# utiasSTARS/pyslam

Hardware: AMD Instinct MI355X
Metric: ms/LM-iter (Jac build + J^T J + Schur solve), stereo BA @ 500k residuals (lower is better)
Workload: dtype f64

## Files before the change

### pyslam_amd/csrc/ps_abi_problem.h

```cpp


const char* ps_last_error(void) { return g_err.c_str(); }

int ps_device_count(void) {
    int n = 0;
    if (hipGetDeviceCount(&n) != hipSuccess) return 0;
    return n;
}

int ps_warm_up(void) {
    static std::once_flag once;
    static int rc = 0;
    std::call_once(once, [] {
        void* p = nullptr;
        if (hipMalloc(&p, 256) != hipSuccess) { rc = fail("hipMalloc failed (no usable HIP device?)"); return; }
        hipLaunchKernelGGL(k_zero4, dim3(1), dim3(256), 0, 0, (size_t)8, (double*)p, (size_t)0, (double*)nullptr, (size_t)0,
                           (double*)nullptr, (size_t)0, (double*)nullptr);
        double hostw[4] = {0, 0, 0, 0};
        (void)hipMemsetAsync(p, 0, 256, 0);
        (void)hipMemcpyAsync((char*)p + 128, p, 64, hipMemcpyDeviceToDevice, 0);
        (void)hipMemcpyAsync(hostw, p, sizeof(hostw), hipMemcpyDeviceToHost, 0);
        if (hipDeviceSynchronize() != hipSuccess) rc = fail("the warm-up launch failed");
        hipFree(p);
        hipFuncAttributes a;
#define PS_TOUCH(...) (void)hipFuncGetAttributes(&a, reinterpret_cast<const void*>(&__VA_ARGS__))
        PS_TOUCH(k_landmark_pass<false>); PS_TOUCH(k_landmark_pass_packed<false, false>); PS_TOUCH(k_landmark_pass_packed<false, true>); PS_TOUCH(k_backsub_packed<false>); PS_TOUCH(k_pose_pass<false>); PS_TOUCH(k_pose_finalize); PS_TOUCH(k_schur_pairs_db<0>);
        PS_TOUCH(k_schur_combine); PS_TOUCH(k_backsub<false>); PS_TOUCH(k_cost_reproj<false>); PS_TOUCH(k_cost_packed<false>); PS_TOUCH(k_reduce3); PS_TOUCH(k_reduce_partials);
        PS_TOUCH(k_copy2); PS_TOUCH(k_zero4); PS_TOUCH(k_lag_status_check);
        PS_TOUCH(k_block_jacobi_factor<6>); PS_TOUCH(k_scale_blocks<6>); PS_TOUCH(k_scale_blocks_p<6>); PS_TOUCH(k_rows_setup<6>);
        PS_TOUCH(k_coarse_rowsums<6>); PS_TOUCH(k_coarse_matrix<6>); PS_TOUCH(k_coarse_chol<6, true>); PS_TOUCH(k_coarse_border<6>);
        PS_TOUCH(k_coarse_mreduce<6>); PS_TOUCH(k_coarse_xbuild<6>); PS_TOUCH(k_coarse_recover<6>); PS_TOUCH(k_cg_fused_lds<6, 8>);
        PS_TOUCH(k_cg_fused<6, 8>); PS_TOUCH(k_cg_unscale<6>); PS_TOUCH(k_update_poses<6>); PS_TOUCH(k_update_points);
        PS_TOUCH(k_xcoarse_rowsums<6>); PS_TOUCH(k_xcoarse_matrix<6>); PS_TOUCH(k_band_chol<6>); PS_TOUCH(k_band_inverse); PS_TOUCH(k_band_inverse_rl<false>);
        PS_TOUCH(k_band_inverse_rl<true>); PS_TOUCH(k_bp_v); PS_TOUCH(k_bp_t); PS_TOUCH(k_bp_w); PS_TOUCH(k_bp_dense_sep); PS_TOUCH(k_bp_dense);
        PS_TOUCH(k_xcg_restrict<6>); PS_TOUCH(k_xcg_f2_coarse<6, 3>); PS_TOUCH(k_xcg_fused1<6, 8, false>); PS_TOUCH(k_xcg_fused1<6, 0, true>);
        PS_TOUCH(k_xcg_fused1<6, 2, false>); PS_TOUCH(k_xcg_fused1<6, 6, false>);
        PS_TOUCH(k_factor_pass<6>); PS_TOUCH(k_factor_assemble<6>); PS_TOUCH(k_cost_factors<6>);
        PS_TOUCH(k_factor_pass<3>); PS_TOUCH(k_factor_assemble<3>); PS_TOUCH(k_cost_factors<3>); PS_TOUCH(k_block_jacobi_factor<3>);
        PS_TOUCH(k_update_poses<3>); PS_TOUCH(k_direct_solve<6>); PS_TOUCH(k_direct_solve<3>);
        PS_TOUCH(k_motion_only_solve<false>); PS_TOUCH(k_motion_only_iteration<false>);
        PS_TOUCH(k_pcg_spmv<6>); PS_TOUCH(k_pcg_spmv<3>); PS_TOUCH(k_ldi_init); PS_TOUCH(k_ldi_update); PS_TOUCH(k_ldi_gemm); PS_TOUCH(k_ldi_mirror);
        PS_TOUCH(k_ldi_ritz); PS_TOUCH(k_ldi_seed_prep); PS_TOUCH(k_ldi_fro_total); PS_TOUCH(k_ldi_pad_identity);
        PS_TOUCH(k_ldi_scaled_dense<6>); PS_TOUCH(k_ldi_sym_unscale<6>); PS_TOUCH(k_ldi_scaled_dense<3>); PS_TOUCH(k_ldi_sym_unscale<3>);
        PS_TOUCH(k_shard_pack<6>); PS_TOUCH(k_shard_unpack<6>); PS_TOUCH(k_publish); PS_TOUCH(k_cov_rhs); PS_TOUCH(k_triangulate<false>);
        PS_TOUCH(k_scale_blocks<3>); PS_TOUCH(k_rows_setup<3>); PS_TOUCH(k_coarse_rowsums<3>); PS_TOUCH(k_coarse_matrix<3>);
        PS_TOUCH(k_coarse_chol<3, true>); PS_TOUCH(k_coarse_border<3>); PS_TOUCH(k_coarse_mreduce<3>); PS_TOUCH(k_coarse_xbuild<3>);
        PS_TOUCH(k_coarse_recover<3>); PS_TOUCH(k_cg_fused_lds<3, 8>); PS_TOUCH(k_cg_unscale<3>);
#undef PS_TOUCH
    });
    return rc;
}

int ps_problem_destroy(ps_problem* h) {
    if (!h) return 0;
    if (h->cp_dbg) {
        long long c[8]; hipMemcpy(c, h->cp_dbg, 64, hipMemcpyDeviceToHost);
        int khz = 100000; hipDeviceGetAttribute(&khz, hipDeviceAttributeWallClockRate, 0);
        fprintf(stderr, "k_cg_persist, workgroup 0, %ld launches, us per launch: recurrences %.2f | sync %.2f | products + publish %.2f | gather %.2f "
                "(%.1f failed passes) | sync %.2f | dots + sync %.2f\n", h->cp_launches, c[0] * 1e3 / khz / h->cp_launches, c[1] * 1e3 / khz / h->cp_launches,
                c[2] * 1e3 / khz / h->cp_launches, c[3] * 1e3 / khz / h->cp_launches, (double)c[7] / h->cp_launches, c[4] * 1e3 / khz / h->cp_launches,
                c[5] * 1e3 / khz / h->cp_launches);
        hipFree(h->cp_dbg);
    }
    if (h->xp_dbg) {
        std::vector<long long> c(3 * 64 * 8); hipMemcpy(c.data(), h->xp_dbg, c.size() * 8, hipMemcpyDeviceToHost);
        int khz = 100000; hipDeviceGetAttribute(&khz, hipDeviceAttributeWallClockRate, 0);
        for (int w = 0; w < 3; ++w) {
            double ph[6] = {0, 0, 0, 0, 0, 0}; int np = 0;
            for (int p = 1; p < 64; ++p) {
                const long long* t = &c[((size_t)w * 64 + p) * 8];
                if (!t[6] || !t[4]) break;
                ph[0] += t[0] - t[6]; ph[1] += t[1] - t[0]; ph[2] += t[2] - t[1]; ph[3] += t[5] - t[2]; ph[4] += t[3] - t[5]; ph[5] += t[4] - t[3]; ++np;
            }
            const double u = 1e3 / khz / std::max(np, 1);
            fprintf(stderr, "k_xcg_persist, workgroup %s, last launch, %d passes, us per pass: t + coarse y %.2f | columns %.2f | products + publish %.2f | "
                    "first gather pass %.2f | rest of the gather %.2f | record sums + dots %.2f | sum %.2f\n", w == 0 ? "0" : (w == 1 ? "nwg/2" : "nwg-1"), np,
                    ph[0] * u, ph[1] * u, ph[2] * u, ph[3] * u, ph[4] * u, ph[5] * u, (ph[0] + ph[1] + ph[2] + ph[3] + ph[4] + ph[5]) * u);
        }
        hipFree(h->xp_dbg);
    }
    if (h->chk_sums) {
        hipDeviceSynchronize();
        fprintf(stderr, "PS_XCG_INV_SUM %p:", (void*)h);
        for (int k = 0; k < std::min(h->chk_nsum, 64); ++k) fprintf(stderr, " [%d use %016llx | side A_c %016llx -> inv %016llx]", k, h->chk_sums[3 * k], h->chk_sums[3 * k + 1], h->chk_sums[3 * k + 2]);
        fprintf(stderr, "\n");
        hipHostFree(h->chk_sums);
    }
    if (h->chk_cnt) {
        int32_t c[4] = {}; hipDeviceSynchronize(); hipMemcpy(c, h->chk_cnt, 16, hipMemcpyDeviceToHost);
        fprintf(stderr, "PS_XCG_AC_CHECK: %d comparisons, entries that differ between the side stream's assembly and the solver stream's: A_c %d, BSZ %d; A_c behind the assembly vs at the end of the side job: %d\n", c[2], c[0], c[1], c[3]);
        hipFree(h->chk_Ac_side); hipFree(h->chk_Ac); hipFree(h->chk_BSZ); hipFree(h->chk_cnt);
    }
    if (ps_env("PS_HOST_TIMING") && h->host_calls)
        fprintf(stderr, "ps_gn_iteration: %ld calls, %.1f us per call on the host, of which %.1f us waiting for the GPU (%ld waits)\n",
                h->host_calls, h->host_call_ns * 1e-3 / h->host_calls, h->host_wait_ns * 1e-3 / h->host_calls, h->host_waits);
    hipStreamSynchronize(h->stream);
    h->persist_release();
    if (h->side) hipStreamSynchronize(h->side);
    if (h->ldi_stream) hipStreamSynchronize(h->ldi_stream);
    cov_release(h);
    if (h->cov_xbuf) hipFree(h->cov_xbuf);
    if (h->tri_buf) hipFree(h->tri_buf);
    for (void* p : h->allocs) hipFree(p);
    h->arena_release();
    for (hipEvent_t e : h->ev_pool) hipEventDestroy(e);
    if (h->ev_ldi) { hipEventDestroy(h->ev_ldi); hipEventDestroy(h->ev_ldi_sread); }
    if (h->ldi_stream && !ps_pool().give(ps_pool().side_streams, h->ldi_stream)) hipStreamDestroy(h->ldi_stream);
    if (h->side) { hipStreamSynchronize(h->side); if (!h->side_poolable || !ps_pool().give(ps_pool().side_streams, h->side)) hipStreamDestroy(h->side); hipEventDestroy(h->ev_ac); hipEventDestroy(h->ev_chol); hipEventDestroy(h->ev_acdone); }
    if (h->own_stream && h->stream && !ps_pool().give(ps_pool().streams, h->stream)) hipStreamDestroy(h->stream);
    delete h;
    return 0;
}

struct DescStage {
    ps_problem_desc d;
    std::vector<std::vector<char>> bufs;
    int pull_bytes(const void** field, size_t bytes) {
        if (!bytes || !*field) return 0;
        bufs.emplace_back(bytes);
        if (hipMemcpy(bufs.back().data(), *field, bytes, hipMemcpyDeviceToHost) != hipSuccess)
            return fail("ps_problem_create: copy of a device-resident table failed (PS_DESC_DEVICE_TABLES set on a host pointer?)");
        *field = bufs.back().data();
        return 0;
    }
    int pull(const double** f, size_t n) { return pull_bytes((const void**)f, n * sizeof(double)); }
    int pull(const int32_t** f, size_t n) { return pull_bytes((const void**)f, n * sizeof(int32_t)); }
    bool obs_pending = false;
    int pull_obs() {
        if (!obs_pending) return 0;
        obs_pending = false;
        const size_t N = (size_t)std::max<int64_t>(0, d.num_obs);
        return pull(&d.obs_pose, N) || pull(&d.obs_point, N) || pull(&d.obs_uvd, 3 * N) || pull(&d.obs_grp, N);
    }
    int stage(const ps_problem_desc* in) {
        d = *in;
        if (!(d.flags & PS_DESC_DEVICE_TABLES)) return 0;
        const size_t P = std::max(0, d.num_poses), L = std::max(0, d.num_points), N = (size_t)std::max<int64_t>(0, d.num_obs);
        const size_t E = (size_t)std::max<int64_t>(0, d.num_edges), Q = (size_t)std::max<int64_t>(0, d.num_priors);
        const size_t X = (size_t)std::max<int64_t>(0, d.num_extra_pairs), PW = d.dof == 6 ? 12 : 6, DD = (size_t)d.dof * d.dof;
        obs_pending = N > 0;
        return pull(&d.pose_rid, P) || pull(&d.point_vid, L) || pull(&d.cams, 5 * (size_t)std::max(0, d.num_cams)) || pull(&d.stiff3, 9 * (size_t)std::max(0, d.num_stiff3)) ||
               pull(&d.obs_groups, 4 * (size_t)std::max(0, d.num_obs_groups)) || pull(&d.e_i, E) || pull(&d.e_j, E) ||
// ... 739 lines not shown
```

### pyslam_amd/csrc/ps_host_cg.h

```cpp

namespace {

struct StageTimer {
    ps_problem* h;
    int stage;
    hipEvent_t a = nullptr, b = nullptr;
    int slot = -1;
    StageTimer(ps_problem* h_, int st, int level = 2) : h(h_), stage(st) {
        if (h->profiling < level) return;
        if (h->profiling == 1 && h->prof_every > 1 &&
            h->prof_tick % h->prof_every != (st == PS_ST_CG_KERNEL ? h->prof_every / 2 : 0)) return;
        if (h->ev_used + 2 > h->ev_pool.size()) {
            for (int i = 0; i < 64; ++i) { hipEvent_t e; hipEventCreate(&e); h->ev_pool.push_back(e); }
        }
        slot = (int)h->ev_used;
        a = h->ev_pool[h->ev_used++];
        b = h->ev_pool[h->ev_used++];
        hipEventRecord(a, h->stream);
    }
    void stop() {
        if (!a) return;
        hipEventRecord(b, h->stream);
        h->pending.push_back({stage, slot});
        a = nullptr;
// ... 626 lines not shown
    if (G) h->Bmat = h->Bmat2[h->lagx_ok ? h->lci_cur : 0];
    hipLaunchKernelGGL(k_block_jacobi_factor<D>, dim3(cdiv(nr, 4)), dim3(256), 0, h->stream, nr, h->diag_slot,
                       h->S, h->Linv, h->status, h->g, h->cg_r[0], h->cg_w[0], h->cg_s[0], h->cg_p, h->cg_xh,
                       h->poses, h->pose_of_rid, h->coarse_basis, G ? h->Bmat : (double*)nullptr, h->bgv);
    hipLaunchKernelGGL(k_scale_blocks<D>, dim3(h->nnzb), dim3(64), 0, h->stream, nr, h->row_ptr, h->col_idx,
                       h->brow_of, h->Linv, h->S, h->aug_slot, h->Saug, G ? h->Bmat : (const double*)nullptr, h->SB);
    if (G) {
        const int ncb = h->ncb, nc = h->nc;
        if (h->side_pending) {
            HIP_OK(hipStreamWaitEvent(h->stream, h->ev_chol, 0));
            h->side_pending = false;
        }
        hipLaunchKernelGGL(k_coarse_rowsums<D>, dim3(nr), dim3(256), (size_t)(ncb + 1) * D * D * sizeof(double), h->stream,
                           nr, ncb, h->run_lo, h->run_hi, h->acol_idx, h->pnode, h->pw0, h->pw1, h->SB, h->SZ, h->Bmat, h->BSZ);
        hipLaunchKernelGGL(k_coarse_matrix<D>, dim3(cdiv((long)ncb * ncb * D * D, 256)), dim3(256), 0, h->stream,
                           nr, ncb, h->slo, h->shi, h->pnode, h->pw0, h->pw1, h->BSZ, h->Ac);
        auto launch_chol = [&](hipStream_t st, int buf, int32_t* stat) -> int { return coarse_factor<D>(h, st, buf, stat); };
        const bool lag = allow_lag && h->coarse_lag && h->lci_next >= 0 && (!h->cg_split || (long)h->nnzb > 24L * nr) &&
                         !(h->lagx_ok && h->lagx);
        if (lag && h->cg_split && !h->Mc && h->alloc(&h->Mc, (size_t)nc * nc)) return -1;
        h->mc_active = lag && h->cg_split;
        const int rpw = nc >= 192 ? 4 : 1;
        const int border_lds = (int)((size_t)rpw * D * nc * sizeof(double));
        if (ensure_dynamic_lds((const void*)k_coarse_border<D>, (size_t)border_lds)) return -1;
        if (lag) {
            const int use = h->lci_next;
            h->lci_cur = use;
            const CoarseRhsArgs ra{h->slo, h->shi, h->pnode, h->pw0, h->pw1, h->LciT2[use], h->tvec, h->cg_r[0], h->cg_w[0],
                                   h->cg_s[0], h->cg_p, h->cg_xh, h->cg_split ? 0 : 2, h->lag_status, h->status, h->bgv, h->cg_split ? h->Mc : nullptr};
            hipLaunchKernelGGL(k_coarse_border<D>, dim3(cdiv(nr, rpw) + ncb + 1), dim3(256), border_lds, h->stream,
                               nr, ncb, h->SZ, h->Lci2[use], h->arow_ptr, h->fine_nnz, h->Saug, h->cg_split ? 0 : 1, h->Ac, ra, rpw);
            HIP_OK(hipEventRecord(h->ev_ac, h->stream));
            HIP_OK(hipStreamWaitEvent(h->side, h->ev_ac, 0));
            if (launch_chol(h->side, use ^ 1, h->lag_status)) return -1;
            HIP_OK(hipEventRecord(h->ev_chol, h->side));
            h->lci_next = use ^ 1; h->side_pending = true;
        } else {
            const int buf = h->lci_cur;
            if (launch_chol(h->stream, buf, h->status)) return -1;
            if (h->lagx_ok)
                hipLaunchKernelGGL(k_coarse_xbuild<D>, dim3(cdiv((long)nr * D * nc, 256)), dim3(256), 0, h->stream, nr, ncb,
                                   h->pnode, h->pw0, h->pw1, h->Bmat, h->Lci2[buf], h->X2[buf]);
            const CoarseRhsArgs ra{h->slo, h->shi, h->pnode, h->pw0, h->pw1, h->LciT2[buf], h->tvec, h->cg_r[0], h->cg_w[0],
                                   h->cg_s[0], h->cg_p, h->cg_xh, h->cg_split ? 0 : 1, nullptr, h->status, h->bgv, nullptr};
            hipLaunchKernelGGL(k_coarse_border<D>, dim3(cdiv(nr, rpw) + 1), dim3(256), border_lds, h->stream,
                               nr, ncb, h->SZ, h->Lci2[buf], h->arow_ptr, h->fine_nnz, h->Saug, h->cg_split ? 0 : 1,
                               (const double*)nullptr, ra, rpw);
            h->lci_next = buf;
        }
    }
    h->cg_launched = 0;
    return 0;
}

template <int D>
int cg_side_kick(ps_problem* h) {
    if (!h->side_todo || !h->side_ready) return 0;
    h->side_todo = false;
    const int nr = h->nr, ncb = h->ncb, nc = h->nc, nb = h->side_buf;
    hipLaunchKernelGGL(k_coarse_rowsums<D>, dim3(nr), dim3(256), (size_t)(ncb + 1) * D * D * sizeof(double), h->side,
                       nr, ncb, h->run_lo, h->run_hi, h->acol_idx, h->pnode, h->pw0, h->pw1, h->SB, h->SZ, h->Bmat2[nb], h->BSZ);
    hipLaunchKernelGGL(k_coarse_matrix<D>, dim3(cdiv((long)ncb * ncb * D * D, 256)), dim3(256), 0, h->side,
                       nr, ncb, h->slo, h->shi, h->pnode, h->pw0, h->pw1, h->BSZ, h->Ac);
    if (coarse_factor<D>(h, h->side, nb, h->lag_status)) return -1;
    hipLaunchKernelGGL(k_coarse_xbuild<D>, dim3(cdiv((long)nr * D * nc, 256)), dim3(256), 0, h->side, nr, ncb,
                       h->pnode, h->pw0, h->pw1, h->Bmat2[nb], h->Lci2[nb], h->X2[nb]);
    HIP_OK(hipEventRecord(h->ev_chol, h->side));
    h->lci_next = nb; h->side_pending = true;
    return 0;
}

int side_kick(ps_problem* h) {
    if (!h->side_todo) return 0;
    return h->D == 6 ? cg_side_kick<6>(h) : cg_side_kick<3>(h);
}

template <int D>
void cg_fused_launch(ps_problem* h, double tol, int count) {
    const int cap = h->hist_cap;
    const int rows = h->cg_split ? h->nr : h->nr_aug;
    const int ncbs = h->cg_split ? h->ncb : 0;
    const double tol2 = tol * tol;
#ifdef PS_MEASURE
    if (ps_env("PS_CP_CLOCKS") && !h->cp_dbg) { hipMalloc(&h->cp_dbg, 64); hipMemset(h->cp_dbg, 0, 64); }
#endif
    if (h->cg_persist && h->cp_ok && h->G > 0 && h->cg_lds && !h->cg_split && !h->cg_two_level_reduce &&
        !h->cg_ablate && h->cg_launched == 0 && h->cg_max_launches > 0 && h->cg_max_launches <= 4090 && !h->no_repeat &&
        h->persist_reserve(h->cp_cus_needed)) {
        const int nl = h->cg_max_launches;
        if (++h->cp_salt >= (1u << 20)) {
            hipMemsetAsync(h->cp_exch, 0, (size_t)4 * h->cp_ntasks * D * sizeof(unsigned long long), h->stream);
            h->cp_salt = 1;
        }
#define PS_CP_LAUNCH(NE) hipLaunchKernelGGL((k_cg_persist<D, NE>), dim3(cdiv(h->cp_ntasks, PS_CP_NT / 64)), dim3(PS_CP_NT), 0, h->stream, h->nr_aug * D, \
                           h->cp_ntasks, (const CpTask*)h->cp_tasks, h->cp_row_task0, h->acol_idx, h->Saug, h->cg_r[0], h->cg_w[0], h->cg_s[0], h->cg_p, \
                           h->cg_xh, h->hist, cap, nl, tol2, h->status, h->scalars, h->cp_exch, h->cp_salt, h->cp_spin, h->cp_dbg,                  \
                           CpRecover{h->nr, h->ncb, h->pnode, h->pw0, h->pw1, h->Linv, h->Lci2[h->lci_cur], h->Bmat, h->x})
        if ((long)h->cp_ntasks * D <= 6L * PS_CP_NT) PS_CP_LAUNCH(6); else PS_CP_LAUNCH(12);
#undef PS_CP_LAUNCH
        h->cg_launched = nl; h->cg_kernel_launches += 1; ++h->cp_launches;
        h->cp_recovered = true;
        return;
    }
    h->cg_kernel_launches += count;
    for (int i = 0; i < count; ++i, ++h->cg_launched) {
        const int n = h->cg_launched, o = n & 1, nw = o ^ 1;
        const double* tot = h->cg_two_level_reduce ? h->cg_tot : nullptr;
        if (tot && !h->cg_split && n > 0)
            hipLaunchKernelGGL(k_cg_reduce, dim3(1), dim3(1024), 0, h->stream, rows, h->cg_gd[o], h->cg_tot, h->status);
#define PS_CG_LAUNCH(NWV)                                                                                          \
        hipLaunchKernelGGL((k_cg_fused<D, NWV>), dim3(rows), dim3(64 * NWV), 0, h->stream, rows, h->arow_ptr,           \
                           h->acol_idx, h->Saug, h->cg_r[o], h->cg_w[o], h->cg_s[o], h->cg_r[nw], h->cg_w[nw],        \
                           h->cg_s[nw], h->cg_p, h->cg_xh, h->cg_gd[o], h->cg_gd[nw], h->hist, cap, n - 1, tol2,      \
                           h->status, h->scalars, h->nr, h->ell_wf, h->ell_wc, h->cg_ablate, tot, ncbs,              \
                           h->fine_nnz, h->cg_cgd[o], h->cg_U, h->cg_ab)
        if (h->cg_lds && !h->cg_short_rows && !h->cg_split && !tot && !h->cg_ablate && rows <= 1024 &&
            (long)rows * D <= PS_CGV_MAX) {
            hipLaunchKernelGGL((k_cg_fused_lds<D, 8>), dim3(rows), dim3(512), 0, h->stream, rows, h->arow_ptr,
                               h->acol_idx, h->Saug, h->cg_r[o], h->cg_w[o], h->cg_s[o], h->cg_r[nw], h->cg_w[nw],
                               h->cg_s[nw], h->cg_p, h->cg_xh, h->cg_gd[o], h->cg_gd[nw], h->hist, cap, n - 1, tol2,
                               h->status, h->scalars, h->nr, h->ell_wf, h->ell_wc);
        }
        else if (h->cg_short_rows) { PS_CG_LAUNCH(1); }
        else if (rows > 1024) { PS_CG_LAUNCH(4); }
        else { PS_CG_LAUNCH(8); }
#undef PS_CG_LAUNCH
        if (h->cg_split)
            hipLaunchKernelGGL(k_cg_reduce_split<D>, dim3(1 + h->ncb), dim3(1024), 0, h->stream, rows, h->ncb,
                               h->cg_gd[nw], h->cg_tot, h->cg_U, h->cg_ab, h->cg_r[o], h->cg_w[o], h->cg_s[o],
                               h->cg_r[nw], h->cg_w[nw], h->cg_s[nw], h->cg_p, h->cg_xh, h->cg_cgd[nw], h->status,
                               h->mc_active ? h->Mc : (const double*)nullptr);
    }
}

template <int D>
void cg_fused_recover(ps_problem* h, const int32_t* gate) {
    const int nr = h->nr;
    if (gate && h->cp_recovered) { h->cp_recovered = false; return; }
    h->cp_recovered = false;
    if (h->G)
        hipLaunchKernelGGL(k_coarse_recover<D>, dim3(cdiv((long)nr * D, 256)), dim3(256), 0, h->stream, nr, h->ncb,
                           h->pnode, h->pw0, h->pw1, h->Linv, h->Lci2[h->lci_cur], h->cg_xh, h->x, gate, h->Bmat);
    else
        hipLaunchKernelGGL(k_cg_unscale<D>, dim3(cdiv((long)nr * D, 256)), dim3(256), 0, h->stream, nr, h->Linv,
                           h->cg_xh, h->x, gate);
}

int cg_report(ps_problem* h, int* iters_out, double* relres_out) {
    h->prev_pcg_iters = h->last_pcg_iters;
    h->last_pcg_iters = h->h_status[ST_PCG_ITERS];
    if (iters_out) *iters_out = h->h_status[ST_PCG_ITERS];
    const double rr0 = h->h_scalars[SC_RR0], rrf = h->h_scalars[SC_RRFINAL];
    if (relres_out) *relres_out = rr0 > 0.0 ? std::sqrt(rrf / rr0) : 0.0;
    if (h->h_status[ST_LM_FAIL]) {
        h->lci_next = -1;
        return fail("a landmark block H_ll is not positive definite");
    }
    if (h->h_status[ST_DIAG_FAIL]) {
        if (h->lag_status) hipMemsetAsync(h->lag_status, 0, ST_NWORDS * sizeof(int32_t), h->stream);
        h->lci_next = -1;
        return fail("reduced system has a non-positive-definite diagonal block (gauge freedom? hold a pose constant or add a prior)");
    }
    if (h->h_status[ST_PCG_DONE] == 2) {
        char buf[200];
        snprintf(buf, sizeof buf, "CG breakdown: the reduced system is not positive definite (iteration %d, relative residual %.2e)",
                 h->h_status[ST_PCG_ITERS], rr0 > 0.0 ? std::sqrt(rrf / rr0) : 0.0);
        return fail(buf);
// ... 362 lines not shown
```

### pyslam_amd/csrc/ps_k_cg_persist.h

```cpp
#pragma once

#define PS_CP_NT 512
#define PS_CP_NQ 6
#define PS_CP_TASKB (8 * PS_CP_NQ)
#define PS_CP_NV 4
#define PS_CP_NE_MAX 12
#define PS_CP_MAXN (PS_CP_NV * PS_CP_NT)
#define PS_PERSIST_TIMEOUT_TICKS 100000000LL
#ifndef PS_CP_SLEEP
#define PS_CP_SLEEP 1
#endif

struct CpTask { int32_t row, b0, b1, pad; };
struct CpRecover { int nr, ncb; const int32_t* pnode; const double *pw0, *pw1, *Linv, *Lci, *Bmat; double* x; };

typedef unsigned long long ps_u64;
typedef __attribute__((address_space(1))) ps_u64 ps_gu64;

typedef unsigned ps_u32x4 __attribute__((ext_vector_type(4)));
PS_DEV void cp_put(ps_u64* g, unsigned tag, double v) {
    const ps_u64 b = (ps_u64)__double_as_longlong(v);
    const ps_u32x4 q = {(unsigned)(b & 0xffffffffull), tag, (unsigned)(b >> 32), tag};
    asm volatile("global_store_dwordx4 %0, %1, off sc1\n\ts_nop 1" :: "v"(g), "v"(q) : "memory");
}

template <int D, int NE>
__global__ __launch_bounds__(PS_CP_NT) void k_cg_persist(
    int n , int ntasks, const CpTask* __restrict__ tasks,
    const int32_t* __restrict__ row_task0 ,
    const int32_t* __restrict__ acol_idx, const double* __restrict__ Saug,
    const double* __restrict__ r0, const double* __restrict__ w0, const double* __restrict__ s0,
    double* __restrict__ p_io, double* __restrict__ x_io,
    double* __restrict__ hist, int cap, int nlaunch , double tol2,
    int32_t* __restrict__ status, double* __restrict__ scalars,
    ps_u64* __restrict__ exch , unsigned salt, unsigned spin_limit,
    long long* __restrict__ dbg , CpRecover rec)
{
    constexpr int DD = D * D;
    __shared__ double rn[PS_CP_MAXN];
    __shared__ double wex[NE * PS_CP_NT];
    __shared__ double red[2][2][PS_CP_NT / 64];
    __shared__ int bad;
    const int t = threadIdx.x, wv = t >> 6, lane = t & 63, kk = lane >> 3, r = lane & 7;
    const int task = blockIdx.x * (PS_CP_NT / 64) + wv;
    const bool chief = blockIdx.x == 0 && t == 0;
    const size_t nex = (size_t)ntasks * D;
    if (t == 0) bad = 0;
    int b0 = 0, b1 = 0;
    if (task < ntasks) { const CpTask tk = tasks[task]; b0 = tk.b0; b1 = tk.b1; }
    int cj[PS_CP_NQ];
    double sv[PS_CP_NQ][D];
#pragma unroll
    for (int q = 0; q < PS_CP_NQ; ++q) {
        const int b = b0 + kk + 8 * q;
        cj[q] = 0;
#pragma unroll
        for (int c = 0; c < D; ++c) sv[q][c] = 0.0;
        if (b < b1 && r < D) {
            cj[q] = acol_idx[b] * D;
            const double* sb = Saug + (size_t)b * DD + r * D;
#pragma unroll
            for (int c = 0; c < D; ++c) sv[q][c] = sb[c];
        }
    }
    double vr[PS_CP_NV], vw[PS_CP_NV], vs[PS_CP_NV], vp[PS_CP_NV], vx[PS_CP_NV];
    int e0[PS_CP_NV], en[PS_CP_NV];
#pragma unroll
    for (int v = 0; v < PS_CP_NV; ++v) {
        const int i = t + v * PS_CP_NT;
        vr[v] = vw[v] = vs[v] = vp[v] = vx[v] = 0.0; e0[v] = 0; en[v] = 0;
        if (i < n) {
            vr[v] = r0[i]; vw[v] = w0[i]; vs[v] = s0[i]; vp[v] = p_io[i]; vx[v] = x_io[i];
            const int row = i / D, ta = row_task0[row];
            e0[v] = ta * D + (i - row * D); en[v] = row_task0[row + 1] - ta;
        }
    }
    if (status[ST_PCG_DONE]) return;
    double gamma = 0.0, delta = 0.0, inv_gprev = 0.0, inv_aprev = 0.0, thresh = 0.0;
    bool converged = false;
    long long ck[8] = {0, 0, 0, 0, 0, 0, 0, 0};
#define PS_CP_CLK(i) do { if (dbg) { const long long now_ = wall_clock64(); ck[i] += now_ - last_; last_ = now_; } } while (0)
    long long last_ = dbg ? wall_clock64() : 0;
    for (int k = -1; k < nlaunch - 1; ++k) {
        double alpha = 0.0, beta = 0.0;
        if (k >= 0) {
            if (k == 0) thresh = tol2 * gamma;
            if (!(gamma > thresh)) {
                if (chief) { status[ST_PCG_DONE] = (gamma != gamma) ? 2 : 1; scalars[SC_RRFINAL] = gamma; if (k == 0) scalars[SC_RR0] = gamma; }
                converged = !(gamma != gamma);
                break;
            }
            beta = (k == 0) ? 0.0 : gamma * inv_gprev;
            const double denom = (k == 0) ? delta : delta - beta * gamma * inv_aprev;
            alpha = gamma / denom;
            if (!(denom > 0.0)) {
                if (chief) { status[ST_PCG_DONE] = 2; scalars[SC_RRFINAL] = gamma; }
                break;
            }
            if (chief) {
                hist[k] = gamma; hist[cap + k] = alpha; status[ST_PCG_ITERS] = k + 1; scalars[SC_RRFINAL] = gamma;
                if (k == 0) { scalars[SC_THRESH] = thresh; scalars[SC_RR0] = gamma; }
            }
        }
        const double gamma_now = gamma, alpha_now = alpha;
        double gs = 0.0;
#pragma unroll
        for (int v = 0; v < PS_CP_NV; ++v) {
            const int i = t + v * PS_CP_NT;
            const double sn = vw[v] + beta * vs[v];
            const double pn = vr[v] + beta * vp[v];
            const double rnv = cg_rnew(vr[v], vw[v], vs[v], alpha, beta);
            vs[v] = sn; vp[v] = pn; vx[v] += alpha * pn; vr[v] = rnv;
            if (i < n) { rn[i] = rnv; gs += rnv * rnv; }
        }
        double (*rd)[PS_CP_NT / 64] = red[k & 1];
        gs = wave_sum(gs);
        if (lane == 0) rd[0][wv] = gs;
        PS_CP_CLK(0);
        __syncthreads();
        PS_CP_CLK(1);
        double gamma_next = 0.0;
#pragma unroll
        for (int w2 = 0; w2 < PS_CP_NT / 64; ++w2) gamma_next += rd[0][w2];
        const unsigned tag = salt * 4096u + (unsigned)(k + 2);
        ps_u64* buf = exch + (size_t)(k & 1) * nex * 2;
        {
            double acc = 0.0;
#pragma unroll
            for (int q = 0; q < PS_CP_NQ; ++q) {
                const double* v = rn + cj[q];
#pragma unroll
                for (int c = 0; c < D; ++c) acc += sv[q][c] * v[c];
            }
            acc += __shfl_xor(acc, 8, 64);
            acc += __shfl_xor(acc, 16, 64);
            acc += __shfl_xor(acc, 32, 64);
            if (task < ntasks && lane < D) cp_put(buf + 2 * ((size_t)task * D + lane), tag, acc);
        }
        if (k >= 0) { inv_gprev = 1.0 / gamma_now; inv_aprev = 1.0 / alpha_now; }
        PS_CP_CLK(2);
        {
            double gv[NE];
            bool ok = false;
            const long long t_enter = (long long)wall_clock64();
            for (unsigned spins = 0; !ok; ++spins) {
                ok = true;
#pragma unroll
                for (int v = 0; v < NE; ++v) {
                    const int j = t + v * PS_CP_NT;
                    gv[v] = 0.0;
                    if (j < (int)nex) {
                        const ps_u64* g = buf + 2 * (size_t)j;
                        const ps_u64 a = __hip_atomic_load((const ps_gu64*)g, __ATOMIC_RELAXED, __HIP_MEMORY_SCOPE_AGENT);
                        const ps_u64 b = __hip_atomic_load((const ps_gu64*)(g + 1), __ATOMIC_RELAXED, __HIP_MEMORY_SCOPE_AGENT);
                        ok = ok && (unsigned)(a >> 32) == tag && (unsigned)(b >> 32) == tag;
                        gv[v] = __longlong_as_double((long long)((a & 0xffffffffull) | (b << 32)));
                    }
                }
                ok = __all(ok);
                if (!ok) {
                    if (spins > spin_limit || (long long)wall_clock64() - t_enter > PS_PERSIST_TIMEOUT_TICKS) { bad = 1; break; }
                    if (PS_CP_SLEEP) __builtin_amdgcn_s_sleep(PS_CP_SLEEP);
                    ck[7] += 1;
                }
            }
#pragma unroll
            for (int v = 0; v < NE; ++v) { const int j = t + v * PS_CP_NT; if (j < (int)nex) wex[j] = gv[v]; }
        }
        PS_CP_CLK(3);
        __syncthreads();
        PS_CP_CLK(4);
#pragma unroll
        for (int v = 0; v < PS_CP_NV; ++v) {
            double wsum = 0.0;
            for (int m = 0; m < en[v]; ++m) wsum += wex[e0[v] + m * D];
            vw[v] = wsum;
        }
        double ds = 0.0;
#pragma unroll
        for (int v = 0; v < PS_CP_NV; ++v) ds += vw[v] * vr[v];
        ds = wave_sum(ds);
        if (lane == 0) rd[1][wv] = ds;
        __syncthreads();
        PS_CP_CLK(5);
        if (bad) {
            if (t == 0) { status[ST_PCG_DONE] = 2; status[ST_PERSIST_FAIL] = 1; }
            break;
        }
        gamma = gamma_next; delta = 0.0;
#pragma unroll
        for (int w2 = 0; w2 < PS_CP_NT / 64; ++w2) delta += rd[1][w2];
    }
    if (dbg && chief) for (int i = 0; i < 8; ++i) dbg[i] += ck[i];
#undef PS_CP_CLK
    if (blockIdx.x == 0) {
        if (converged && rec.x) {
            const int nc = rec.ncb * D, nf = rec.nr * D;
            __syncthreads();
#pragma unroll
            for (int v = 0; v < PS_CP_NV; ++v) { const int i = t + v * PS_CP_NT; if (i < n) rn[i] = vx[v]; }
            __syncthreads();
            const double* xc = rn + nf;
            for (int base = 0; base < nc; base += PS_CP_NT / 8) {
                const int kq = base + t / 8, sub = t & 7;
                double v = 0.0;
                if (kq < nc) for (int m = kq + sub; m < nc; m += 8) v += rec.Lci[(size_t)m * nc + kq] * xc[m];
                v += __shfl_xor(v, 1, 64); v += __shfl_xor(v, 2, 64); v += __shfl_xor(v, 4, 64);
                if (kq < nc && sub == 0) wex[kq] = v;
            }
            __syncthreads();
            for (int e = t; e < nf; e += PS_CP_NT) {
                const int i = e / D, c = e - i * D, q = rec.pnode[i];
                const double w0 = rec.pw0[i], w1 = rec.pw1[i];
                double z[D];
#pragma unroll
                for (int m = 0; m < D; ++m) z[m] = w0 * wex[q * D + m] + ((q + 1 < rec.ncb) ? w1 * wex[(q + 1) * D + m] : 0.0);
                double v = 0.0;
#pragma unroll
                for (int a = 0; a < D; ++a) {
                    double xhat = rn[i * D + a];
#pragma unroll
                    for (int m = 0; m < D; ++m) xhat += rec.Bmat[(size_t)i * DD + a * D + m] * z[m];
                    v += rec.Linv[(size_t)i * DD + a * D + c] * xhat;
                }
                rec.x[e] = v;
            }
        }
#pragma unroll
        for (int v = 0; v < PS_CP_NV; ++v) {
            const int i = t + v * PS_CP_NT;
            if (i < n) { x_io[i] = vx[v]; p_io[i] = vp[v]; }
        }
    }
}
```

### pyslam_amd/csrc/ps_k_packed.h

```cpp
#pragma once

#define PS_LMW_MAXOBS 16

__global__ __launch_bounds__(256) void k_lmw_maxobs(int nv, const int32_t* __restrict__ lm_ptr, int32_t* __restrict__ out) {
    const int v = blockIdx.x * blockDim.x + threadIdx.x;
    const int n = v < nv ? lm_ptr[v + 1] - lm_ptr[v] : -1;
    int mx = n, mn = n < 0 ? INT_MAX : n;
    for (int off = 32; off; off >>= 1) { mx = max(mx, __shfl_xor(mx, off, 64)); mn = min(mn, __shfl_xor(mn, off, 64)); }
    if ((threadIdx.x & 63) == 0 && mx >= 0) { atomicMax(out, mx); atomicMin(out + 1, mn); }
}

__global__ __launch_bounds__(256) void k_lmw_items(int nv, int nwaves, int W, const int32_t* __restrict__ lm_ptr, int32_t* __restrict__ first) {
    const int w = blockIdx.x * blockDim.x + threadIdx.x;
    if (w > nwaves) return;
    if (w == nwaves) { first[w] = nv; return; }
    const int target = W * w;
    int lo = 0, hi = nv;
    while (lo < hi) { const int mid = (lo + hi) >> 1; if (lm_ptr[mid] < target) lo = mid + 1; else hi = mid; }
    first[w] = lo;
}

struct LmwSeg { int v, lane0, lane1, nrows, row0; bool valid, head; };
PS_DEV LmwSeg lmw_segment(int v0, int v1, const int32_t* __restrict__ lm_ptr, int lane, volatile int32_t* flags ) {
    LmwSeg s;
// ... 136 lines not shown
            lm_emit_m(ev, M[0], M[1], M[2], M[3], M[4], M[5], z);
            z[9] = ev.pc[0]; z[10] = ev.pc[1]; z[11] = ev.pc[2];
            z[12] = (double)rid_of_obs;
        }
        double2* dst = reinterpret_cast<double2*>(sm + PS_ZROW * lane);
#pragma unroll
        for (int k = 0; k < PS_ZROW / 2; ++k) dst[k] = make_double2(z[2 * k], z[2 * k + 1]);
    }
    __builtin_amdgcn_wave_barrier();
    const double2* src = reinterpret_cast<const double2*>(sm);
    double2* out = reinterpret_cast<double2*>(Z + PS_ZROW * (size_t)sg.row0);
    for (int k = lane; k < sg.nrows * (PS_ZROW / 2); k += 64) out[k] = src[k];
    }
    if (COST) {
        obs_cost = block_sum(obs_cost, csum);
        if (threadIdx.x == 0) cost_part[blockIdx.x] = obs_cost;
    }
}

template <bool WIDE>
__global__ __launch_bounds__(256) void k_cost_packed(
    int nwaves, const int32_t* __restrict__ lmw_first, const int32_t* __restrict__ lm_ptr, const int32_t* __restrict__ lm_point,
    const LObs* __restrict__ lobs, const double* __restrict__ poses, const double* __restrict__ points,
    const ObsGroup* __restrict__ groups, double* __restrict__ cost_part, const int32_t* __restrict__ gate, ObsWide wide)
{
    __shared__ double csum[16];
    if (gate && gate[ST_PCG_DONE] != 1) return;
    const int lane = threadIdx.x & 63, wv = threadIdx.x >> 6, gw = blockIdx.x * 4 + wv;
    double c = 0.0;
    const int v0 = gw < nwaves ? lmw_first[gw] : 0, v1 = gw < nwaves ? lmw_first[gw + 1] : 0;
    if (v1 > v0) {
        const int row0 = lm_ptr[v0], nrows = lm_ptr[v1] - row0;
        if (lane < nrows) {
            const int i = row0 + lane;
            const LObs o = lobs[i];
            const Se3 T = se3_load(poses + 12 * PS_POSE_OF(o));
            const double pw[3] = {points[3 * (size_t)o.point], points[3 * (size_t)o.point + 1], points[3 * (size_t)o.point + 2]};
            ReprojEval ev;
            reproj_eval_obs<false, false, WIDE>(T, pw, &o.u, groups, PS_GRP_OF(o), wide, i, ev);
            c = ev.cost;
        }
    }
    c = block_sum(c, csum);
    if (threadIdx.x == 0) cost_part[blockIdx.x] = c;
}

template <bool MD>
__global__ __launch_bounds__(256) void k_backsub_packed(
    int nwaves, const int32_t* __restrict__ lmw_first, const int32_t* __restrict__ lm_ptr,
    const double* __restrict__ Z, const double* __restrict__ Cinv, const double* __restrict__ cvec,
    const double* __restrict__ xp, double* __restrict__ dxl,
    double* __restrict__ sq_part ,
    const int32_t* __restrict__ gate,
    int nblk_l, const int32_t* __restrict__ lm_point, double* __restrict__ points,
    int P, const int32_t* __restrict__ pose_rid, double* __restrict__ poses, double* __restrict__ sq_part_p,
    long long* __restrict__ hearly, long long eseq, double* __restrict__ md_part = nullptr, double lam_ratio = 0.0)
{
    __shared__ double lds[16];
    __shared__ double sm3[4][64 * 3];
    __shared__ int32_t flags[4][64];
    const bool closed = gate && gate[ST_PCG_DONE] != 1;
    if (hearly && blockIdx.x == 0 && threadIdx.x == 0) *reinterpret_cast<volatile long long*>(hearly) = closed ? -eseq : eseq;
    if (closed) return;
    if ((int)blockIdx.x >= nblk_l) {
        typedef PoseOps<6> G;
        const int i = (blockIdx.x - nblk_l) * blockDim.x + threadIdx.x;
        double sq = 0.0;
        const int rid = (i < P) ? pose_rid[i] : -1;
        if (rid >= 0) {
            double xi[6];
#pragma unroll
            for (int k = 0; k < 6; ++k) { xi[k] = xp[(size_t)rid * 6 + k]; sq += xi[k] * xi[k]; }
            G::store(poses + G::W * (size_t)i, G::mul(G::exp(xi), G::load(poses + G::W * (size_t)i)));
        }
        sq = block_sum(sq, lds);
        if (threadIdx.x == 0) sq_part_p[blockIdx.x - nblk_l] = sq;
        return;
    }
    const int lane = threadIdx.x & 63, wv = threadIdx.x >> 6, gw = blockIdx.x * 4 + wv;
    double sq = 0.0, md = 0.0;
    const int v0 = gw < nwaves ? lmw_first[gw] : 0, v1 = gw < nwaves ? lmw_first[gw + 1] : 0;
    if (v1 > v0) {
        const LmwSeg sg = lmw_segment(v0, v1, lm_ptr, lane, flags[wv]);
        double a0 = 0.0, a1 = 0.0, a2 = 0.0;
        if (sg.valid) {
            const double2* zq = reinterpret_cast<const double2*>(Z + PS_ZROW * (size_t)(sg.row0 + lane));
            double z[14];
#pragma unroll
            for (int k = 0; k < 7; ++k) { const double2 t = zq[k]; z[2 * k] = t.x; z[2 * k + 1] = t.y; }
            const int rid = (int)z[12];
            if (rid >= 0) {
                const double* x = xp + 6 * (size_t)rid;
                const double y0 = x[0] - (z[10] * x[5] - z[11] * x[4]);
                const double y1 = x[1] - (z[11] * x[3] - z[9] * x[5]);
                const double y2 = x[2] - (z[9] * x[4] - z[10] * x[3]);
                a0 = -(z[0] * y0 + z[3] * y1 + z[6] * y2);
                a1 = -(z[1] * y0 + z[4] * y1 + z[7] * y2);
                a2 = -(z[2] * y0 + z[5] * y1 + z[8] * y2);
            }
        }
        double* sm = sm3[wv];
        sm[3 * lane] = a0; sm[3 * lane + 1] = a1; sm[3 * lane + 2] = a2;
        __builtin_amdgcn_wave_barrier();
        if (sg.head) {
            double b0 = 0.0, b1 = 0.0, b2 = 0.0;
            for (int l = lane; l < sg.lane1; ++l) { b0 += sm[3 * l]; b1 += sm[3 * l + 1]; b2 += sm[3 * l + 2]; }
            const size_t v = (size_t)sg.v;
            const double* m = Cinv + 6 * v;
            b0 += cvec[3 * v]; b1 += cvec[3 * v + 1]; b2 += cvec[3 * v + 2];
            const double d0 = m[0] * b0 + m[1] * b1 + m[3] * b2;
            const double d1 = m[2] * b1 + m[4] * b2;
            const double d2 = m[5] * b2;
            dxl[3 * v] = d0; dxl[3 * v + 1] = d1; dxl[3 * v + 2] = d2;
            sq = d0 * d0 + d1 * d1 + d2 * d2;
            if (MD) md = lm_landmark_terms(m, cvec + 3 * v, d0, d1, d2, lam_ratio);
            if (points) {
                double* pt = points + 3 * (size_t)lm_point[v];
                pt[0] += d0; pt[1] += d1; pt[2] += d2;
            }
        }
    }
    sq = block_sum(sq, lds);
    if (threadIdx.x == 0) sq_part[blockIdx.x] = sq;
    if (MD) {
        md = block_sum(md, lds);
        if (threadIdx.x == 0) md_part[blockIdx.x] = md;
    }
}
```

Before: 0.3006.

## Hoist loads ahead of branches and spread CG solution recovery across all workgroups

The persistent CG kernel now issues its entry loads (vectors, row-task bounds, Saug blocks, column indices) unconditionally with clamped indices, so they can overlap before the done-check. The final recovery of the full solution, previously done by workgroup 0 alone, now runs in every workgroup: each recomputes the small coarse product and writes its own slice of rows. The landmark-update kernel likewise loads Z rows, Cinv, cvec and point coordinates before the branch. Debug clock slots for prologue and epilogue are added. The trade-off is redundant coarse work per workgroup and extra loads on lanes that would have been idle.

Measured after the change: 0.3157. 1.05x slower.

```diff
diff --git a/pyslam_amd/csrc/ps_abi_problem.h b/pyslam_amd/csrc/ps_abi_problem.h
--- a/pyslam_amd/csrc/ps_abi_problem.h
+++ b/pyslam_amd/csrc/ps_abi_problem.h
@@ -54,10 +54,11 @@
 int ps_problem_destroy(ps_problem* h) {
     if (!h) return 0;
     if (h->cp_dbg) {
-        long long c[8]; hipMemcpy(c, h->cp_dbg, 64, hipMemcpyDeviceToHost);
+        long long c[PS_CP_NCLK]; hipMemcpy(c, h->cp_dbg, sizeof(c), hipMemcpyDeviceToHost);
         int khz = 100000; hipDeviceGetAttribute(&khz, hipDeviceAttributeWallClockRate, 0);
-        fprintf(stderr, "k_cg_persist, workgroup 0, %ld launches, us per launch: recurrences %.2f | sync %.2f | products + publish %.2f | gather %.2f "
-                "(%.1f failed passes) | sync %.2f | dots + sync %.2f\n", h->cp_launches, c[0] * 1e3 / khz / h->cp_launches, c[1] * 1e3 / khz / h->cp_launches,
+        fprintf(stderr, "k_cg_persist, workgroup 0, %ld launches, us per launch: prologue %.2f | epilogue %.2f | recurrences %.2f | sync %.2f | products + publish %.2f | gather %.2f "
+                "(%.1f failed passes) | sync %.2f | dots + sync %.2f\n", h->cp_launches, c[6] * 1e3 / khz / h->cp_launches, c[8] * 1e3 / khz / h->cp_launches,
+                c[0] * 1e3 / khz / h->cp_launches, c[1] * 1e3 / khz / h->cp_launches,
                 c[2] * 1e3 / khz / h->cp_launches, c[3] * 1e3 / khz / h->cp_launches, (double)c[7] / h->cp_launches, c[4] * 1e3 / khz / h->cp_launches,
                 c[5] * 1e3 / khz / h->cp_launches);
         hipFree(h->cp_dbg);
diff --git a/pyslam_amd/csrc/ps_host_cg.h b/pyslam_amd/csrc/ps_host_cg.h
--- a/pyslam_amd/csrc/ps_host_cg.h
+++ b/pyslam_amd/csrc/ps_host_cg.h
@@ -732,7 +732,7 @@
     const int ncbs = h->cg_split ? h->ncb : 0;
     const double tol2 = tol * tol;
 #ifdef PS_MEASURE
-    if (ps_env("PS_CP_CLOCKS") && !h->cp_dbg) { hipMalloc(&h->cp_dbg, 64); hipMemset(h->cp_dbg, 0, 64); }
+    if (ps_env("PS_CP_CLOCKS") && !h->cp_dbg) { hipMalloc(&h->cp_dbg, PS_CP_NCLK * 8); hipMemset(h->cp_dbg, 0, PS_CP_NCLK * 8); }
 #endif
     if (h->cg_persist && h->cp_ok && h->G > 0 && h->cg_lds && !h->cg_split && !h->cg_two_level_reduce &&
         !h->cg_ablate && h->cg_launched == 0 && h->cg_max_launches > 0 && h->cg_max_launches <= 4090 && !h->no_repeat &&
diff --git a/pyslam_amd/csrc/ps_k_cg_persist.h b/pyslam_amd/csrc/ps_k_cg_persist.h
--- a/pyslam_amd/csrc/ps_k_cg_persist.h
+++ b/pyslam_amd/csrc/ps_k_cg_persist.h
@@ -6,6 +6,7 @@
 #define PS_CP_NV 4
 #define PS_CP_NE_MAX 12
 #define PS_CP_MAXN (PS_CP_NV * PS_CP_NT)
+#define PS_CP_NCLK 9
 #define PS_PERSIST_TIMEOUT_TICKS 100000000LL
 #ifndef PS_CP_SLEEP
 #define PS_CP_SLEEP 1
@@ -46,47 +47,65 @@
     const bool chief = blockIdx.x == 0 && t == 0;
     const size_t nex = (size_t)ntasks * D;
     if (t == 0) bad = 0;
-    int b0 = 0, b1 = 0;
-    if (task < ntasks) { const CpTask tk = tasks[task]; b0 = tk.b0; b1 = tk.b1; }
+    long long ck[PS_CP_NCLK] = {0, 0, 0, 0, 0, 0, 0, 0, 0};
+#define PS_CP_CLK(i) do { if (dbg) { const long long now_ = wall_clock64(); ck[i] += now_ - last_; last_ = now_; } } while (0)
+    long long last_ = dbg ? wall_clock64() : 0;
+    const int done_at_entry = status[ST_PCG_DONE];
+    const CpTask tk = tasks[min(task, ntasks - 1)];
+    const int b0 = task < ntasks ? tk.b0 : 0, b1 = task < ntasks ? tk.b1 : 0;
+    double vr[PS_CP_NV], vw[PS_CP_NV], vs[PS_CP_NV], vp[PS_CP_NV], vx[PS_CP_NV];
+    int e0[PS_CP_NV], en[PS_CP_NV];
+    {
+        int ta[PS_CP_NV], tb[PS_CP_NV];
+#pragma unroll
+        for (int v = 0; v < PS_CP_NV; ++v) {
+            const int ic = min(t + v * PS_CP_NT, n - 1), row = ic / D;
+            vr[v] = r0[ic]; vw[v] = w0[ic]; vs[v] = s0[ic]; vp[v] = p_io[ic]; vx[v] = x_io[ic];
+            ta[v] = row_task0[row]; tb[v] = row_task0[row + 1];
+        }
+#pragma unroll
+        for (int v = 0; v < PS_CP_NV; ++v) {
+            const int i = t + v * PS_CP_NT;
+            const bool in = i < n;
+            if (!in) vr[v] = vw[v] = vs[v] = vp[v] = vx[v] = 0.0;
+            e0[v] = in ? ta[v] * D + (i - (i / D) * D) : 0; en[v] = in ? tb[v] - ta[v] : 0;
+        }
+    }
     int cj[PS_CP_NQ];
     double sv[PS_CP_NQ][D];
-#pragma unroll
-    for (int q = 0; q < PS_CP_NQ; ++q) {
-        const int b = b0 + kk + 8 * q;
-        cj[q] = 0;
-#pragma unroll
-        for (int c = 0; c < D; ++c) sv[q][c] = 0.0;
-        if (b < b1 && r < D) {
-            cj[q] = acol_idx[b] * D;
-            const double* sb = Saug + (size_t)b * DD + r * D;
+    {
+        const int rc = r < D ? r : D - 1;
+        int bq[PS_CP_NQ];
+#pragma unroll
+        for (int q = 0; q < PS_CP_NQ; ++q) { const int b = b0 + kk + 8 * q; bq[q] = b < b1 ? b : 0; }
+#pragma unroll
+        for (int q = 0; q < PS_CP_NQ; ++q) cj[q] = acol_idx[bq[q]];
+#pragma unroll
+        for (int q = 0; q < PS_CP_NQ; ++q) {
+            const double* sb = Saug + (size_t)bq[q] * DD + rc * D;
 #pragma unroll
             for (int c = 0; c < D; ++c) sv[q][c] = sb[c];
         }
-    }
-    double vr[PS_CP_NV], vw[PS_CP_NV], vs[PS_CP_NV], vp[PS_CP_NV], vx[PS_CP_NV];
-    int e0[PS_CP_NV], en[PS_CP_NV];
-#pragma unroll
-    for (int v = 0; v < PS_CP_NV; ++v) {
-        const int i = t + v * PS_CP_NT;
-        vr[v] = vw[v] = vs[v] = vp[v] = vx[v] = 0.0; e0[v] = 0; en[v] = 0;
-        if (i < n) {
-            vr[v] = r0[i]; vw[v] = w0[i]; vs[v] = s0[i]; vp[v] = p_io[i]; vx[v] = x_io[i];
-            const int row = i / D, ta = row_task0[row];
-            e0[v] = ta * D + (i - row * D); en[v] = row_task0[row + 1] - ta;
-        }
-    }
-    if (status[ST_PCG_DONE]) return;
+#pragma unroll
+        for (int q = 0; q < PS_CP_NQ; ++q) {
+            const bool live = b0 + kk + 8 * q < b1 && r < D;
+            cj[q] = live ? cj[q] * D : 0;
+#pragma unroll
+            for (int c = 0; c < D; ++c) sv[q][c] = live ? sv[q][c] : 0.0;
+        }
+    }
+    if (done_at_entry) return;
     double gamma = 0.0, delta = 0.0, inv_gprev = 0.0, inv_aprev = 0.0, thresh = 0.0;
     bool converged = false;
-    long long ck[8] = {0, 0, 0, 0, 0, 0, 0, 0};
-#define PS_CP_CLK(i) do { if (dbg) { const long long now_ = wall_clock64(); ck[i] += now_ - last_; last_ = now_; } } while (0)
-    long long last_ = dbg ? wall_clock64() : 0;
+#ifdef PS_MEASURE
+    if (dbg) { asm volatile("s_waitcnt vmcnt(0) lgkmcnt(0)" ::: "memory"); const long long now_ = wall_clock64(); ck[6] = now_ - last_; last_ = now_; }
+#endif
     for (int k = -1; k < nlaunch - 1; ++k) {
         double alpha = 0.0, beta = 0.0;
         if (k >= 0) {
             if (k == 0) thresh = tol2 * gamma;
             if (!(gamma > thresh)) {
-                if (chief) { status[ST_PCG_DONE] = (gamma != gamma) ? 2 : 1; scalars[SC_RRFINAL] = gamma; if (k == 0) scalars[SC_RR0] = gamma; }
+                if (chief) { atomicMax(&status[ST_PCG_DONE], (gamma != gamma) ? 2 : 1); scalars[SC_RRFINAL] = gamma; if (k == 0) scalars[SC_RR0] = gamma; }
                 converged = !(gamma != gamma);
                 break;
             }
@@ -184,52 +203,57 @@
         __syncthreads();
         PS_CP_CLK(5);
         if (bad) {
-            if (t == 0) { status[ST_PCG_DONE] = 2; status[ST_PERSIST_FAIL] = 1; }
+            if (t == 0) { atomicMax(&status[ST_PCG_DONE], 2); status[ST_PERSIST_FAIL] = 1; }
             break;
         }
         gamma = gamma_next; delta = 0.0;
 #pragma unroll
         for (int w2 = 0; w2 < PS_CP_NT / 64; ++w2) delta += rd[1][w2];
     }
-    if (dbg && chief) for (int i = 0; i < 8; ++i) dbg[i] += ck[i];
-#undef PS_CP_CLK
+    if (converged && rec.x) {
+        const int nc = rec.ncb * D, nf = rec.nr * D;
+        __syncthreads();
+#pragma unroll
+        for (int v = 0; v < PS_CP_NV; ++v) { const int i = t + v * PS_CP_NT; if (i < n) rn[i] = vx[v]; }
+        __syncthreads();
+        const double* xc = rn + nf;
+        for (int base = 0; base < nc; base += PS_CP_NT / 8) {
+            const int kq = base + t / 8, sub = t & 7;
+            double v = 0.0;
+            if (kq < nc) for (int m = kq + sub; m < nc; m += 8) v += rec.Lci[(size_t)m * nc + kq] * xc[m];
+            v += __shfl_xor(v, 1, 64); v += __shfl_xor(v, 2, 64); v += __shfl_xor(v, 4, 64);
+            if (kq < nc && sub == 0) wex[kq] = v;
+        }
+        __syncthreads();
+        const int per = (nf + (int)gridDim.x - 1) / (int)gridDim.x;
+        const int e_lo = (int)blockIdx.x * per, e_hi = min(nf, e_lo + per);
+        for (int e = e_lo + t; e < e_hi; e += PS_CP_NT) {
+            const int i = e / D, c = e - i * D, q = rec.pnode[i];
+            const double w0 = rec.pw0[i], w1 = rec.pw1[i];
+            double z[D];
+#pragma unroll
+            for (int m = 0; m < D; ++m) z[m] = w0 * wex[q * D + m] + ((q + 1 < rec.ncb) ? w1 * wex[(q + 1) * D + m] : 0.0);
+            double v = 0.0;
+#pragma unroll
+            for (int a = 0; a < D; ++a) {
+                double xhat = rn[i * D + a];
+#pragma unroll
+                for (int m = 0; m < D; ++m) xhat += rec.Bmat[(size_t)i * DD + a * D + m] * z[m];
+                v += rec.Linv[(size_t)i * DD + a * D + c] * xhat;
+            }
+            rec.x[e] = v;
+        }
+    }
     if (blockIdx.x == 0) {
-        if (converged && rec.x) {
-            const int nc = rec.ncb * D, nf = rec.nr * D;
-            __syncthreads();
-#pragma unroll
-            for (int v = 0; v < PS_CP_NV; ++v) { const int i = t + v * PS_CP_NT; if (i < n) rn[i] = vx[v]; }
-            __syncthreads();
-            const double* xc = rn + nf;
-            for (int base = 0; base < nc; base += PS_CP_NT / 8) {
-                const int kq = base + t / 8, sub = t & 7;
-                double v = 0.0;
-                if (kq < nc) for (int m = kq + sub; m < nc; m += 8) v += rec.Lci[(size_t)m * nc + kq] * xc[m];
-                v += __shfl_xor(v, 1, 64); v += __shfl_xor(v, 2, 64); v += __shfl_xor(v, 4, 64);
-                if (kq < nc && sub == 0) wex[kq] = v;
-            }
-            __syncthreads();
-            for (int e = t; e < nf; e += PS_CP_NT) {
-                const int i = e / D, c = e - i * D, q = rec.pnode[i];
-                const double w0 = rec.pw0[i], w1 = rec.pw1[i];
-                double z[D];
-#pragma unroll
-                for (int m = 0; m < D; ++m) z[m] = w0 * wex[q * D + m] + ((q + 1 < rec.ncb) ? w1 * wex[(q + 1) * D + m] : 0.0);
-                double v = 0.0;
-#pragma unroll
-                for (int a = 0; a < D; ++a) {
-                    double xhat = rn[i * D + a];
-#pragma unroll
-                    for (int m = 0; m < D; ++m) xhat += rec.Bmat[(size_t)i * DD + a * D + m] * z[m];
-                    v += rec.Linv[(size_t)i * DD + a * D + c] * xhat;
-                }
-                rec.x[e] = v;
-            }
-        }
 #pragma unroll
         for (int v = 0; v < PS_CP_NV; ++v) {
             const int i = t + v * PS_CP_NT;
             if (i < n) { x_io[i] = vx[v]; p_io[i] = vp[v]; }
         }
     }
+#ifdef PS_MEASURE
+    if (dbg) { asm volatile("s_waitcnt vmcnt(0) lgkmcnt(0)" ::: "memory"); PS_CP_CLK(8); }
+#endif
+    if (dbg && chief) for (int i = 0; i < PS_CP_NCLK; ++i) dbg[i] += ck[i];
+#undef PS_CP_CLK
 }
diff --git a/pyslam_amd/csrc/ps_k_packed.h b/pyslam_amd/csrc/ps_k_packed.h
--- a/pyslam_amd/csrc/ps_k_packed.h
+++ b/pyslam_amd/csrc/ps_k_packed.h
@@ -242,42 +242,47 @@
     const int v0 = gw < nwaves ? lmw_first[gw] : 0, v1 = gw < nwaves ? lmw_first[gw + 1] : 0;
     if (v1 > v0) {
         const LmwSeg sg = lmw_segment(v0, v1, lm_ptr, lane, flags[wv]);
+        const double2* zq = reinterpret_cast<const double2*>(Z + PS_ZROW * (size_t)(sg.row0 + min(lane, sg.nrows - 1)));
+        double z[14];
+#pragma unroll
+        for (int k = 0; k < 7; ++k) { const double2 t = zq[k]; z[2 * k] = t.x; z[2 * k + 1] = t.y; }
+        const size_t v = (size_t)min(sg.v, v1 - 1);
+        const int pt = points ? lm_point[v] : 0;
         double a0 = 0.0, a1 = 0.0, a2 = 0.0;
-        if (sg.valid) {
-            const double2* zq = reinterpret_cast<const double2*>(Z + PS_ZROW * (size_t)(sg.row0 + lane));
-            double z[14];
-#pragma unroll
-            for (int k = 0; k < 7; ++k) { const double2 t = zq[k]; z[2 * k] = t.x; z[2 * k + 1] = t.y; }
-            const int rid = (int)z[12];
-            if (rid >= 0) {
-                const double* x = xp + 6 * (size_t)rid;
-                const double y0 = x[0] - (z[10] * x[5] - z[11] * x[4]);
-                const double y1 = x[1] - (z[11] * x[3] - z[9] * x[5]);
-                const double y2 = x[2] - (z[9] * x[4] - z[10] * x[3]);
-                a0 = -(z[0] * y0 + z[3] * y1 + z[6] * y2);
-                a1 = -(z[1] * y0 + z[4] * y1 + z[7] * y2);
-                a2 = -(z[2] * y0 + z[5] * y1 + z[8] * y2);
-            }
+        const int rid = sg.valid ? (int)z[12] : -1;
+        if (rid >= 0) {
+            const double* x = xp + 6 * (size_t)rid;
+            const double y0 = x[0] - (z[10] * x[5] - z[11] * x[4]);
+            const double y1 = x[1] - (z[11] * x[3] - z[9] * x[5]);
+            const double y2 = x[2] - (z[9] * x[4] - z[10] * x[3]);
+            a0 = -(z[0] * y0 + z[3] * y1 + z[6] * y2);
+            a1 = -(z[1] * y0 + z[4] * y1 + z[7] * y2);
+            a2 = -(z[2] * y0 + z[5] * y1 + z[8] * y2);
         }
         double* sm = sm3[wv];
         sm[3 * lane] = a0; sm[3 * lane + 1] = a1; sm[3 * lane + 2] = a2;
         __builtin_amdgcn_wave_barrier();
         if (sg.head) {
+            double m[6], cv[3], pw[3] = {0.0, 0.0, 0.0};
+#pragma unroll
+            for (int k = 0; k < 6; ++k) m[k] = Cinv[6 * v + k];
+#pragma unroll
+            for (int k = 0; k < 3; ++k) cv[k] = cvec[3 * v + k];
+            double* po = points + 3 * (size_t)pt;
+            if (points) {
+#pragma unroll
+                for (int k = 0; k < 3; ++k) pw[k] = po[k];
+            }
             double b0 = 0.0, b1 = 0.0, b2 = 0.0;
             for (int l = lane; l < sg.lane1; ++l) { b0 += sm[3 * l]; b1 += sm[3 * l + 1]; b2 += sm[3 * l + 2]; }
-            const size_t v = (size_t)sg.v;
-            const double* m = Cinv + 6 * v;
-            b0 += cvec[3 * v]; b1 += cvec[3 * v + 1]; b2 += cvec[3 * v + 2];
+            b0 += cv[0]; b1 += cv[1]; b2 += cv[2];
             const double d0 = m[0] * b0 + m[1] * b1 + m[3] * b2;
             const double d1 = m[2] * b1 + m[4] * b2;
             const double d2 = m[5] * b2;
             dxl[3 * v] = d0; dxl[3 * v + 1] = d1; dxl[3 * v + 2] = d2;
             sq = d0 * d0 + d1 * d1 + d2 * d2;
-            if (MD) md = lm_landmark_terms(m, cvec + 3 * v, d0, d1, d2, lam_ratio);
-            if (points) {
-                double* pt = points + 3 * (size_t)lm_point[v];
-                pt[0] += d0; pt[1] += d1; pt[2] += d2;
-            }
+            if (MD) md = lm_landmark_terms(m, cv, d0, d1, d2, lam_ratio);
+            if (points) { po[0] = pw[0] + d0; po[1] = pw[1] + d1; po[2] = pw[2] + d2; }
         }
     }
     sq = block_sum(sq, lds);
```
